# barbararoessle/e2e_multi_view_matching

Measured on NVIDIA H100. Metric: view-tuples/sec @1024 kpts 5-view, higher is better.
Workload: dtype f32 via split operands on the tensor cores (fp16x3 / tf32x3, fp32-faithful) / f64 pose kernels

## Files before the change

e2e_multi_view_matching_b200/csrc/attention_h3.cu:

```cuda
#include "attention_wg.cuh"

int g_attn_h3_variant = 1;
extern "C" void mvm_debug_set_attention_h3_variant(int v) { g_attn_h3_variant = v ? 1 : 0; }

int launch_attention_h3(const float* qkv, const __half* kh, const __half* kl, const __half* vh, const __half* vl,
                        float* out, int batch, int n_pad, AttnSegs segs, int is_cross, cudaStream_t stream) {
  MVM_REQUIRE(qkv && kh && kl && vh && vl && out);
  MVM_REQUIRE(n_pad % 64 == 0 && attn_segs_valid(segs, n_pad, is_cross));
  MvmProfScope prof__(MVM_TAG_ATTN, stream);
  const long long rows = (long long)batch * segs.n_views * n_pad;
  const CUtensorMap* tK = mvm_get_tmap_2d_f16(kh, rows, 256, 256, attn_wg::Cfg<16>::BKV);
  const CUtensorMap* tKlo = mvm_get_tmap_2d_f16(kl, rows, 256, 256, attn_wg::Cfg<16>::BKV);
  const CUtensorMap* tV = mvm_get_tmap_2d_f16(vh, rows, 256, 256, attn_wg::Cfg<16>::BKV);
  const CUtensorMap* tVlo = mvm_get_tmap_2d_f16(vl, rows, 256, 256, attn_wg::Cfg<16>::BKV);
  return attn_wg::launch<16>(tK, tV, tKlo, tVlo, qkv, out, batch, n_pad, segs, is_cross, stream);
}
```

e2e_multi_view_matching_b200/csrc/attention_tc.cu:

```cuda
#include "attention_wg.cuh"

long long* g_attn_dbg = nullptr;

extern "C" void mvm_debug_set_attention_timing(long long* buf) { g_attn_dbg = buf; }

int launch_attention_tc(const float* qkv, const float* vt, float* out, int batch, int n_pad, AttnSegs segs,
                        int is_cross, int n_pass, cudaStream_t stream, const float* klo, const float* vtlo) {
  MVM_REQUIRE(n_pad % 64 == 0 && attn_segs_valid(segs, n_pad, is_cross));
  MvmProfScope prof__(MVM_TAG_ATTN, stream);
  const int V = batch * segs.n_views;
  const long long rows = (long long)V * n_pad;
  const CUtensorMap* tK = mvm_get_tmap_2d(qkv, rows, 768, 768, attn_wg::Cfg<1>::BKV);
  const CUtensorMap* tV = mvm_get_tmap_2d(vt, (long long)V * 256, n_pad, n_pad, attn_wg::HD);
  if (n_pass == 3) {
    MVM_REQUIRE(klo && vtlo);
    const CUtensorMap* tKlo = mvm_get_tmap_2d(klo, rows, 256, 256, attn_wg::Cfg<1>::BKV);
    const CUtensorMap* tVlo = mvm_get_tmap_2d(vtlo, (long long)V * 256, n_pad, n_pad, attn_wg::HD);
    return attn_wg::launch<3>(tK, tV, tKlo, tVlo, qkv, out, batch, n_pad, segs, is_cross, stream);
  }
  return attn_wg::launch<1>(tK, tV, tK, tV, qkv, out, batch, n_pad, segs, is_cross, stream);
}
```

e2e_multi_view_matching_b200/csrc/attention_wg.cuh:

```cuda
#pragma once
#include <cuda_fp16.h>
#include "common.cuh"
#include "kernels.cuh"
#include "tc_common.cuh"

namespace attn_wg {

constexpr int BQ = 128, HD = 64;
constexpr int PRODUCER_WARP = 8;
constexpr int NTHREADS = 384;
constexpr int PRODUCER_REGS = 40, CONSUMER_REGS = 232;
constexpr int PP_BAR = 1;

template <int MODE>
struct Cfg {
  static constexpr bool F16 = MODE == 16;
  static constexpr bool PIPE = F16;
  static constexpr int BKV = F16 ? 128 : 64;
  static constexpr int PL = MODE == 1 ? 1 : 2;
  static constexpr int PLANE = 16384;
  static constexpr int TILE = PL * PLANE;
  static constexpr int ST = MODE == 1 ? 4 : 3;
  static constexpr int OFF_V = ST * TILE;
  static constexpr int OFF_BAR = 2 * ST * TILE;
  static constexpr int SMEM_BYTES = OFF_BAR + 256 + 1024;
};

struct Args {
  const float* qkv;
  float* out;
  int n_pad;
  AttnSegs segs;
  int is_cross;
};

__device__ __forceinline__ float ex2_ftz(float x) {
  float y;
  asm("ex2.approx.ftz.f32 %0, %1;" : "=f"(y) : "f"(x));
  return y;
}
__device__ __forceinline__ float tf32_hi(float x) {
  return __uint_as_float((__float_as_uint(x) + 0x1000u) & 0xffffe000u);
}
__device__ __forceinline__ void split_pack(float x0, float x1, uint32_t& hi, uint32_t& lo) {
  const __half2 h = __floats2half2_rn(x0, x1);
  const float2 hf = __half22float2(h);
  const __half2 l = __floats2half2_rn(x0 - hf.x, x1 - hf.y);
  hi = *reinterpret_cast<const uint32_t*>(&h);
  lo = *reinterpret_cast<const uint32_t*>(&l);
}
__device__ __forceinline__ void named_bar_sync(int id, int n) {
  asm volatile("bar.sync %0, %1;" ::"r"(id), "r"(n) : "memory");
}
__device__ __forceinline__ void named_bar_arrive(int id, int n) {
  asm volatile("bar.arrive %0, %1;" ::"r"(id), "r"(n) : "memory");
}
template <int N>
__device__ __forceinline__ void fence_regs(uint32_t (*a)[4]) {
#pragma unroll
  for (int i = 0; i < N; ++i)
#pragma unroll
    for (int e = 0; e < 4; ++e) asm volatile("" : "+r"(a[i][e])::"memory");
}

template <int MODE>
__global__ void __launch_bounds__(NTHREADS, 1)
attention_wg_kernel(const __grid_constant__ CUtensorMap tmK, const __grid_constant__ CUtensorMap tmV,
                    const __grid_constant__ CUtensorMap tmKlo, const __grid_constant__ CUtensorMap tmVlo,
                    const __grid_constant__ Args g) {
  using C_ = Cfg<MODE>;
  constexpr bool F16 = C_::F16, PIPE = C_::PIPE;
  constexpr int ST = C_::ST, PLANE = C_::PLANE, TILE = C_::TILE, BKV = C_::BKV;
  constexpr int KS = F16 ? 4 : 8;
  constexpr int KP = BKV / (F16 ? 16 : 8);
  constexpr int NSC = BKV / 2;
  extern __shared__ uint8_t smem_raw[];
  uint8_t* smem = reinterpret_cast<uint8_t*>((reinterpret_cast<uintptr_t>(smem_raw) + 1023) & ~uintptr_t(1023));
  uint64_t* bars = reinterpret_cast<uint64_t*>(smem + C_::OFF_BAR);
  uint64_t* k_full = bars;
  uint64_t* k_empty = bars + ST;
  uint64_t* v_full = bars + 2 * ST;
  uint64_t* v_empty = bars + 3 * ST;

  const int warp = threadIdx.x >> 5, lane = threadIdx.x & 31;
  const int q0 = blockIdx.x * BQ;
  const int h = blockIdx.y;
  const int v = blockIdx.z;
  const int T = g.segs.n_views;
  const int t = v % T, b = v / T;
  if (q0 >= g.segs.counts[t]) return;

  if (threadIdx.x == 0) {
    for (int i = 0; i < ST; ++i) {
      tc::mbar_init(k_full + i, 1); tc::mbar_init(k_empty + i, 256);
      tc::mbar_init(v_full + i, 1); tc::mbar_init(v_empty + i, 256);
    }
    tc::fence_barrier_init();
  }
  __syncthreads();

  if (warp >= PRODUCER_WARP) {
    asm volatile("setmaxnreg.dec.sync.aligned.u32 %0;" ::"n"(PRODUCER_REGS));
    if (warp == PRODUCER_WARP && lane == 0) {
      tc::prefetch_tmap(&tmK); tc::prefetch_tmap(&tmV);
      if (MODE != 1) { tc::prefetch_tmap(&tmKlo); tc::prefetch_tmap(&tmVlo); }
      int j = 0;
      for (int sg = 0; sg < T; ++sg) {
        if (g.is_cross ? (sg == t) : (sg != t)) continue;
        const int cnt = g.segs.counts[sg];
        for (int k0 = 0; k0 < cnt; k0 += BKV, ++j) {
          const int s = j % ST;
          const uint32_t ph = ((j / ST) & 1) ^ 1;
          const int krow = (b * T + sg) * g.n_pad + k0;
          uint8_t* sk = smem + s * TILE;
          uint8_t* sv = smem + C_::OFF_V + s * TILE;
          tc::mbar_wait(k_empty + s, ph);
          tc::mbar_arrive_expect_tx(k_full + s, TILE);
          if (F16) {
            tc::tma_load_2d(sk, &tmK, k_full + s, h * HD, krow);
            tc::tma_load_2d(sk + PLANE, &tmKlo, k_full + s, h * HD, krow);
          } else {
            tc::tma_load_2d(sk, &tmK, k_full + s, 256 + h * HD, krow);
            tc::tma_load_2d(sk + 8192, &tmK, k_full + s, 256 + h * HD + 32, krow);
            if (MODE == 3) {
              tc::tma_load_2d(sk + PLANE, &tmKlo, k_full + s, h * HD, krow);
              tc::tma_load_2d(sk + PLANE + 8192, &tmKlo, k_full + s, h * HD + 32, krow);
            }
          }
          tc::mbar_wait(v_empty + s, ph);
          tc::mbar_arrive_expect_tx(v_full + s, TILE);
          if (F16) {
            tc::tma_load_2d(sv, &tmV, v_full + s, h * HD, krow);
            tc::tma_load_2d(sv + PLANE, &tmVlo, v_full + s, h * HD, krow);
          } else {
            const int vrow = (b * T + sg) * 256 + h * HD;
            tc::tma_load_2d(sv, &tmV, v_full + s, k0, vrow);
            tc::tma_load_2d(sv + 8192, &tmV, v_full + s, k0 + 32, vrow);
            if (MODE == 3) {
              tc::tma_load_2d(sv + PLANE, &tmVlo, v_full + s, k0, vrow);
              tc::tma_load_2d(sv + PLANE + 8192, &tmVlo, v_full + s, k0 + 32, vrow);
            }
          }
        }
      }
    }
    return;
  }

  asm volatile("setmaxnreg.inc.sync.aligned.u32 %0;" ::"n"(CONSUMER_REGS));
  const int wg = warp >> 2, wq = warp & 3;
  const int gr = lane >> 2, tq = lane & 3;
  const int lrow = wg * 64 + wq * 16 + gr;
  float2 qraw[KS][4];
  {
    const long long total = (long long)gridDim.z * g.n_pad;
    const long long r0 = (long long)v * g.n_pad + q0 + lrow;
    const float* q_r0 = g.qkv + r0 * 768 + h * HD;
    const float* q_r1 = q_r0 + 8 * 768;
    const bool in0 = r0 < total, in1 = r0 + 8 < total;
    const float2 z = make_float2(0.f, 0.f);
#pragma unroll
    for (int kk = 0; kk < KS; ++kk) {
      if (F16) {
        const int c = 16 * kk + 2 * tq;
        qraw[kk][0] = in0 ? __ldg(reinterpret_cast<const float2*>(q_r0 + c)) : z;
        qraw[kk][1] = in1 ? __ldg(reinterpret_cast<const float2*>(q_r1 + c)) : z;
        qraw[kk][2] = in0 ? __ldg(reinterpret_cast<const float2*>(q_r0 + c + 8)) : z;
        qraw[kk][3] = in1 ? __ldg(reinterpret_cast<const float2*>(q_r1 + c + 8)) : z;
      } else {
        const int c = 8 * kk + tq;
        qraw[kk][0] = make_float2(in0 ? __ldg(q_r0 + c) : 0.f, 0.f);
        qraw[kk][1] = make_float2(in1 ? __ldg(q_r1 + c) : 0.f, 0.f);
        qraw[kk][2] = make_float2(in0 ? __ldg(q_r0 + c + 4) : 0.f, 0.f);
        qraw[kk][3] = make_float2(in1 ? __ldg(q_r1 + c + 4) : 0.f, 0.f);
      }
    }
  }
  uint32_t qhi[KS][4], qlo[KS][4];
  if constexpr (F16) {
#pragma unroll
    for (int kk = 0; kk < KS; ++kk)
#pragma unroll
      for (int e = 0; e < 4; ++e) split_pack(qraw[kk][e].x, qraw[kk][e].y, qhi[kk][e], qlo[kk][e]);
  }

  float o[32];
#pragma unroll
  for (int i = 0; i < 32; ++i) o[i] = 0.f;
  float m_run[2] = {-INFINITY, -INFINITY}, l_run[2] = {0.f, 0.f};
  const float scale_l2e = 0.125f * 1.4426950408889634f;
  const int srcA = (lane & ~3) | (tq >> 1), srcB = srcA + 2;
  float sc[NSC], fo[2];
  uint32_t phi[KP][4], plo[KP][4];

  auto prep_s = [&] {
    if constexpr (!F16) {
#pragma unroll
      for (int kk = 0; kk < KS; ++kk) {
#pragma unroll
        for (int e = 0; e < 4; ++e) {
          float x = qraw[kk][e].x;
          asm volatile("" : "+f"(x));
          const float hi = MODE == 3 ? tf32_hi(x) : x;
          qhi[kk][e] = __float_as_uint(hi);
          qlo[kk][e] = __float_as_uint(MODE == 3 ? tf32_hi(x - hi) : 0.f);
        }
      }
    }
#pragma unroll
    for (int i = 0; i < NSC; ++i) sc[i] = 0.f;
    tc::fence_acc<BKV>(sc);
  };
  auto issue_s = [&](int st, uint32_t ph) {
    tc::mbar_wait(k_full + st, ph);
    const uint32_t kb = tc::smem_u32(smem + st * TILE);
    tc::wgmma_fence();
#pragma unroll
    for (int kk = 0; kk < KS; ++kk) {
      if (F16) {
        const uint64_t dk = tc::make_sw128_desc(kb + kk * 32);
        tc::wgmma_f16_rs<BKV, 0>(sc, qhi[kk], dk);
        tc::wgmma_f16_rs<BKV, 0>(sc, qhi[kk], tc::make_sw128_desc(kb + PLANE + kk * 32));
        tc::wgmma_f16_rs<BKV, 0>(sc, qlo[kk], dk);
      } else {
        const uint32_t off = (kk >> 2) * 8192 + (kk & 3) * 32;
        const uint64_t dk = tc::make_sw128_desc(kb + off);
        tc::wgmma_tf32_rs<64>(sc, qhi[kk], dk);
        if (MODE == 3) {
          tc::wgmma_tf32_rs<64>(sc, qhi[kk], tc::make_sw128_desc(kb + PLANE + off));
          tc::wgmma_tf32_rs<64>(sc, qlo[kk], dk);
        }
      }
    }
    tc::wgmma_commit();
  };
  auto retire_s = [&](int st) {
    tc::fence_acc<BKV>(sc);
    fence_regs<KS>(qhi);
    fence_regs<KS>(qlo);
    tc::mbar_arrive(k_empty + st);
  };
  auto issue_pv = [&](int st, uint32_t ph) {
    tc::mbar_wait(v_full + st, ph);
    const uint32_t vb = tc::smem_u32(smem + C_::OFF_V + st * TILE);
    tc::wgmma_fence();
#pragma unroll
    for (int kk = 0; kk < KP; ++kk) {
      if (F16) {
        const uint64_t dv = tc::make_sw128_desc(vb + kk * 2048);
        tc::wgmma_f16_rs<64, 1>(o, phi[kk], dv);
        tc::wgmma_f16_rs<64, 1>(o, phi[kk], tc::make_sw128_desc(vb + PLANE + kk * 2048));
        tc::wgmma_f16_rs<64, 1>(o, plo[kk], dv);
      } else {
        const uint32_t off = (kk >> 2) * 8192 + (kk & 3) * 32;
        const uint64_t dv = tc::make_sw128_desc(vb + off);
        tc::wgmma_tf32_rs<64>(o, phi[kk], dv);
        if (MODE == 3) {
          tc::wgmma_tf32_rs<64>(o, phi[kk], tc::make_sw128_desc(vb + PLANE + off));
          tc::wgmma_tf32_rs<64>(o, plo[kk], dv);
        }
      }
    }
    tc::wgmma_commit();
  };
  auto retire_pv = [&](int st) {
    tc::fence_acc<64>(o);
    fence_regs<KP>(phi);
    fence_regs<KP>(plo);
    tc::mbar_arrive(v_empty + st);
  };
  auto softmax = [&](int nvalid) {
    if (nvalid < BKV) {
#pragma unroll
      for (int i = 0; i < BKV / 8; ++i) {
        const int key = 8 * i + 2 * tq;
        if (key >= nvalid) { sc[4 * i] = -INFINITY; sc[4 * i + 2] = -INFINITY; }
        if (key + 1 >= nvalid) { sc[4 * i + 1] = -INFINITY; sc[4 * i + 3] = -INFINITY; }
      }
    }
#pragma unroll
    for (int hh = 0; hh < 2; ++hh) {
      float mx = sc[2 * hh];
#pragma unroll
      for (int i = 0; i < BKV / 8; ++i) mx = fmaxf(mx, fmaxf(sc[4 * i + 2 * hh], sc[4 * i + 2 * hh + 1]));
      mx = fmaxf(mx, __shfl_xor_sync(0xffffffffu, mx, 1));
      mx = fmaxf(mx, __shfl_xor_sync(0xffffffffu, mx, 2));
      mx *= scale_l2e;
      fo[hh] = 1.f;
      if (mx > m_run[hh] + 8.f) {
        fo[hh] = ex2_ftz(m_run[hh] - mx);
        m_run[hh] = mx;
        l_run[hh] *= fo[hh];
      }
      const float nm = 7.f - m_run[hh];
      float rs = 0.f;
#pragma unroll
      for (int i = 0; i < BKV / 8; ++i) {
        const float p0 = ex2_ftz(fmaf(sc[4 * i + 2 * hh], scale_l2e, nm));
        const float p1 = ex2_ftz(fmaf(sc[4 * i + 2 * hh + 1], scale_l2e, nm));
        sc[4 * i + 2 * hh] = p0;
        sc[4 * i + 2 * hh + 1] = p1;
        rs += p0 + p1;
      }
      l_run[hh] += rs;
    }
  };
  auto rescale_o = [&] {
#pragma unroll
    for (int hh = 0; hh < 2; ++hh) {
      if (fo[hh] != 1.f) {
#pragma unroll
        for (int i = 0; i < 8; ++i) {
          o[4 * i + 2 * hh] *= fo[hh];
          o[4 * i + 2 * hh + 1] *= fo[hh];
        }
      }
    }
  };
  auto split_p = [&] {
#pragma unroll
    for (int kk = 0; kk < KP; ++kk) {
      if (F16) {
#pragma unroll
        for (int e = 0; e < 4; ++e) split_pack(sc[8 * kk + 2 * e], sc[8 * kk + 2 * e + 1], phi[kk][e], plo[kk][e]);
      } else {
        float a[4];
        const bool odd = tq & 1;
        const float x0 = __shfl_sync(0xffffffffu, sc[4 * kk], srcA), x1 = __shfl_sync(0xffffffffu, sc[4 * kk + 1], srcA);
        const float y0 = __shfl_sync(0xffffffffu, sc[4 * kk + 2], srcA), y1 = __shfl_sync(0xffffffffu, sc[4 * kk + 3], srcA);
        const float z0 = __shfl_sync(0xffffffffu, sc[4 * kk], srcB), z1 = __shfl_sync(0xffffffffu, sc[4 * kk + 1], srcB);
        const float w0 = __shfl_sync(0xffffffffu, sc[4 * kk + 2], srcB), w1 = __shfl_sync(0xffffffffu, sc[4 * kk + 3], srcB);
        a[0] = odd ? x1 : x0; a[1] = odd ? y1 : y0; a[2] = odd ? z1 : z0; a[3] = odd ? w1 : w0;
#pragma unroll
        for (int e = 0; e < 4; ++e) {
          const float hi = MODE == 3 ? tf32_hi(a[e]) : a[e];
          phi[kk][e] = __float_as_uint(hi);
          plo[kk][e] = __float_as_uint(a[e] - hi);
        }
      }
    }
  };

  auto finish_pv = [&](int jn) {
    tc::wgmma_wait<0>();
    tc::fence_acc<64>(o);
    fence_regs<KP>(phi);
    fence_regs<KP>(plo);
    if (jn >= 2) tc::mbar_arrive(v_empty + (jn - 2) % ST);
    if (jn >= 1) {
      rescale_o();
      split_p();
    }
  };
  if (PIPE && wg == 1) named_bar_arrive(PP_BAR + 0, 256);
  int j = 0;
  for (int sg = 0; sg < T; ++sg) {
    if (g.is_cross ? (sg == t) : (sg != t)) continue;
    const int cnt = g.segs.counts[sg];
    for (int k0 = 0; k0 < cnt; k0 += BKV, ++j) {
      const int nvalid = cnt - k0;
      const int s = j % ST;
      const uint32_t ph = (j / ST) & 1;
      if constexpr (PIPE) {
        finish_pv(j);
        prep_s();
        named_bar_sync(PP_BAR + wg, 256);
        if (j == 0) {
          issue_s(s, ph);
          named_bar_arrive(PP_BAR + (wg ^ 1), 256);
          tc::wgmma_wait<0>();
        } else {
          issue_s(s, ph);
          issue_pv((j - 1) % ST, ((j - 1) / ST) & 1);
          named_bar_arrive(PP_BAR + (wg ^ 1), 256);
          tc::wgmma_wait<1>();
        }
        retire_s(s);
        softmax(nvalid);
      } else {
        prep_s();
        issue_s(s, ph);
        tc::wgmma_wait<0>();
        retire_s(s);
        softmax(nvalid);
        rescale_o();
        split_p();
        issue_pv(s, ph);
        tc::wgmma_wait<0>();
        retire_pv(s);
      }
    }
  }
  if constexpr (PIPE) {
    finish_pv(j);
    named_bar_sync(PP_BAR + wg, 256);
    if (j > 0) issue_pv((j - 1) % ST, ((j - 1) / ST) & 1);
    if (wg == 0) named_bar_arrive(PP_BAR + 1, 256);
    tc::wgmma_wait<0>();
    if (j > 0) retire_pv((j - 1) % ST);
  }

#pragma unroll
  for (int hh = 0; hh < 2; ++hh) {
    float l = l_run[hh];
    l += __shfl_xor_sync(0xffffffffu, l, 1);
    l += __shfl_xor_sync(0xffffffffu, l, 2);
    const float inv = 1.f / l;
    const int r = lrow + 8 * hh;
    if (q0 + r < g.n_pad) {
      float* op = g.out + ((long long)v * g.n_pad + q0 + r) * 256 + h * HD + 2 * tq;
#pragma unroll
      for (int i = 0; i < 8; ++i)
        *reinterpret_cast<float2*>(op + 8 * i) = make_float2(o[4 * i + 2 * hh] * inv, o[4 * i + 2 * hh + 1] * inv);
    }
  }
}

template <int MODE>
int launch(const CUtensorMap* tK, const CUtensorMap* tV, const CUtensorMap* tKlo, const CUtensorMap* tVlo, const float* qkv,
           float* out, int batch, int n_pad, const AttnSegs& segs, int is_cross, cudaStream_t stream) {
  using C_ = Cfg<MODE>;
  if (!tK || !tV || !tKlo || !tVlo) return MVM_ERR_LAUNCH;
  mvm_once_per_device(MODE == 16 ? MVM_ONCE_ATTN_H3 : MVM_ONCE_ATTN_TC + 16 * (MODE == 3), [&] {
    cudaFuncSetAttribute(attention_wg_kernel<MODE>, cudaFuncAttributeMaxDynamicSharedMemorySize, C_::SMEM_BYTES);
  });
  Args g;
  g.qkv = qkv; g.out = out; g.n_pad = n_pad; g.segs = segs; g.is_cross = is_cross;
  dim3 grid(mvm_div_up(n_pad, BQ), 4, batch * segs.n_views);
  attention_wg_kernel<MODE><<<grid, NTHREADS, C_::SMEM_BYTES, stream>>>(*tK, *tV, *tKlo, *tVlo, g);
  MVM_CHECK_LAUNCH();
  return MVM_OK;
}

}
```

Baseline: 215.3.

## Make attention kernel persistent with TMA-loaded Q tiles and cross-item KV pipelining

Replaces the one-CTA-per-(query block, head, view) grid with a persistent grid sized to the SM count that strides over work items. Q tiles are now fetched by the producer warp via TMA into a swizzled shared buffer instead of per-thread global loads. The K/V stage counter runs continuously across items, so loads for the next item can overlap the previous item's tail, and the final PV of one item is drained before the next begins. This is meant to remove launch/tail waves and Q-load latency. In exchange it adds shared memory and extra barrier bookkeeping, and static round-robin item assignment may load-balance poorly across uneven segments.

```diff
diff --git a/e2e_multi_view_matching_b200/csrc/attention_h3.cu b/e2e_multi_view_matching_b200/csrc/attention_h3.cu
--- a/e2e_multi_view_matching_b200/csrc/attention_h3.cu
+++ b/e2e_multi_view_matching_b200/csrc/attention_h3.cu
@@ -13,5 +13,6 @@
   const CUtensorMap* tKlo = mvm_get_tmap_2d_f16(kl, rows, 256, 256, attn_wg::Cfg<16>::BKV);
   const CUtensorMap* tV = mvm_get_tmap_2d_f16(vh, rows, 256, 256, attn_wg::Cfg<16>::BKV);
   const CUtensorMap* tVlo = mvm_get_tmap_2d_f16(vl, rows, 256, 256, attn_wg::Cfg<16>::BKV);
-  return attn_wg::launch<16>(tK, tV, tKlo, tVlo, qkv, out, batch, n_pad, segs, is_cross, stream);
+  const CUtensorMap* tQ = mvm_get_tmap_2d(qkv, rows, 768, 768, attn_wg::BQ);
+  return attn_wg::launch<16>(tK, tV, tKlo, tVlo, tQ, qkv, out, batch, n_pad, segs, is_cross, stream);
 }
diff --git a/e2e_multi_view_matching_b200/csrc/attention_tc.cu b/e2e_multi_view_matching_b200/csrc/attention_tc.cu
--- a/e2e_multi_view_matching_b200/csrc/attention_tc.cu
+++ b/e2e_multi_view_matching_b200/csrc/attention_tc.cu
@@ -12,11 +12,12 @@
   const long long rows = (long long)V * n_pad;
   const CUtensorMap* tK = mvm_get_tmap_2d(qkv, rows, 768, 768, attn_wg::Cfg<1>::BKV);
   const CUtensorMap* tV = mvm_get_tmap_2d(vt, (long long)V * 256, n_pad, n_pad, attn_wg::HD);
+  const CUtensorMap* tQ = mvm_get_tmap_2d(qkv, rows, 768, 768, attn_wg::BQ);
   if (n_pass == 3) {
     MVM_REQUIRE(klo && vtlo);
     const CUtensorMap* tKlo = mvm_get_tmap_2d(klo, rows, 256, 256, attn_wg::Cfg<1>::BKV);
     const CUtensorMap* tVlo = mvm_get_tmap_2d(vtlo, (long long)V * 256, n_pad, n_pad, attn_wg::HD);
-    return attn_wg::launch<3>(tK, tV, tKlo, tVlo, qkv, out, batch, n_pad, segs, is_cross, stream);
+    return attn_wg::launch<3>(tK, tV, tKlo, tVlo, tQ, qkv, out, batch, n_pad, segs, is_cross, stream);
   }
-  return attn_wg::launch<1>(tK, tV, tK, tV, qkv, out, batch, n_pad, segs, is_cross, stream);
+  return attn_wg::launch<1>(tK, tV, tK, tV, tQ, qkv, out, batch, n_pad, segs, is_cross, stream);
 }
diff --git a/e2e_multi_view_matching_b200/csrc/attention_wg.cuh b/e2e_multi_view_matching_b200/csrc/attention_wg.cuh
--- a/e2e_multi_view_matching_b200/csrc/attention_wg.cuh
+++ b/e2e_multi_view_matching_b200/csrc/attention_wg.cuh
@@ -22,8 +22,11 @@
   static constexpr int TILE = PL * PLANE;
   static constexpr int ST = MODE == 1 ? 4 : 3;
   static constexpr int OFF_V = ST * TILE;
-  static constexpr int OFF_BAR = 2 * ST * TILE;
+  static constexpr int OFF_Q = 2 * ST * TILE;
+  static constexpr int QBOX = BQ * 32 * 4;
+  static constexpr int OFF_BAR = OFF_Q + 2 * QBOX;
   static constexpr int SMEM_BYTES = OFF_BAR + 256 + 1024;
+  static_assert(SMEM_BYTES <= 232448, "attention: dynamic shared memory above the sm_90 opt-in");
 };
 
 struct Args {
@@ -32,7 +35,20 @@
   int n_pad;
   AttnSegs segs;
   int is_cross;
+  int n_qb;
+  int n_items;
 };
+
+struct Item { int q0, h, v, t, b; };
+__device__ __forceinline__ bool item_at(const Args& g, int it, Item& w) {
+  const int r = it / g.n_qb;
+  w.q0 = (it - r * g.n_qb) * BQ;
+  w.h = r & 3;
+  w.v = r >> 2;
+  w.t = w.v % g.segs.n_views;
+  w.b = w.v / g.segs.n_views;
+  return w.q0 < g.segs.counts[w.t];
+}
 
 __device__ __forceinline__ float ex2_ftz(float x) {
   float y;
@@ -67,34 +83,33 @@
 __global__ void __launch_bounds__(NTHREADS, 1)
 attention_wg_kernel(const __grid_constant__ CUtensorMap tmK, const __grid_constant__ CUtensorMap tmV,
                     const __grid_constant__ CUtensorMap tmKlo, const __grid_constant__ CUtensorMap tmVlo,
-                    const __grid_constant__ Args g) {
+                    const __grid_constant__ CUtensorMap tmQ, const __grid_constant__ Args g) {
   using C_ = Cfg<MODE>;
   constexpr bool F16 = C_::F16, PIPE = C_::PIPE;
-  constexpr int ST = C_::ST, PLANE = C_::PLANE, TILE = C_::TILE, BKV = C_::BKV;
+  constexpr int ST = C_::ST, PLANE = C_::PLANE, TILE = C_::TILE, BKV = C_::BKV, QBOX = C_::QBOX;
   constexpr int KS = F16 ? 4 : 8;
   constexpr int KP = BKV / (F16 ? 16 : 8);
   constexpr int NSC = BKV / 2;
   extern __shared__ uint8_t smem_raw[];
   uint8_t* smem = reinterpret_cast<uint8_t*>((reinterpret_cast<uintptr_t>(smem_raw) + 1023) & ~uintptr_t(1023));
+  uint8_t* sq = smem + C_::OFF_Q;
   uint64_t* bars = reinterpret_cast<uint64_t*>(smem + C_::OFF_BAR);
   uint64_t* k_full = bars;
   uint64_t* k_empty = bars + ST;
   uint64_t* v_full = bars + 2 * ST;
   uint64_t* v_empty = bars + 3 * ST;
+  uint64_t* q_full = bars + 4 * ST;
+  uint64_t* q_empty = bars + 4 * ST + 1;
 
   const int warp = threadIdx.x >> 5, lane = threadIdx.x & 31;
-  const int q0 = blockIdx.x * BQ;
-  const int h = blockIdx.y;
-  const int v = blockIdx.z;
   const int T = g.segs.n_views;
-  const int t = v % T, b = v / T;
-  if (q0 >= g.segs.counts[t]) return;
 
   if (threadIdx.x == 0) {
     for (int i = 0; i < ST; ++i) {
       tc::mbar_init(k_full + i, 1); tc::mbar_init(k_empty + i, 256);
       tc::mbar_init(v_full + i, 1); tc::mbar_init(v_empty + i, 256);
     }
+    tc::mbar_init(q_full, 1); tc::mbar_init(q_empty, 256);
     tc::fence_barrier_init();
   }
   __syncthreads();
@@ -102,43 +117,51 @@
   if (warp >= PRODUCER_WARP) {
     asm volatile("setmaxnreg.dec.sync.aligned.u32 %0;" ::"n"(PRODUCER_REGS));
     if (warp == PRODUCER_WARP && lane == 0) {
-      tc::prefetch_tmap(&tmK); tc::prefetch_tmap(&tmV);
+      tc::prefetch_tmap(&tmK); tc::prefetch_tmap(&tmV); tc::prefetch_tmap(&tmQ);
       if (MODE != 1) { tc::prefetch_tmap(&tmKlo); tc::prefetch_tmap(&tmVlo); }
-      int j = 0;
-      for (int sg = 0; sg < T; ++sg) {
-        if (g.is_cross ? (sg == t) : (sg != t)) continue;
-        const int cnt = g.segs.counts[sg];
-        for (int k0 = 0; k0 < cnt; k0 += BKV, ++j) {
-          const int s = j % ST;
-          const uint32_t ph = ((j / ST) & 1) ^ 1;
-          const int krow = (b * T + sg) * g.n_pad + k0;
-          uint8_t* sk = smem + s * TILE;
-          uint8_t* sv = smem + C_::OFF_V + s * TILE;
-          tc::mbar_wait(k_empty + s, ph);
-          tc::mbar_arrive_expect_tx(k_full + s, TILE);
-          if (F16) {
-            tc::tma_load_2d(sk, &tmK, k_full + s, h * HD, krow);
-            tc::tma_load_2d(sk + PLANE, &tmKlo, k_full + s, h * HD, krow);
-          } else {
-            tc::tma_load_2d(sk, &tmK, k_full + s, 256 + h * HD, krow);
-            tc::tma_load_2d(sk + 8192, &tmK, k_full + s, 256 + h * HD + 32, krow);
-            if (MODE == 3) {
-              tc::tma_load_2d(sk + PLANE, &tmKlo, k_full + s, h * HD, krow);
-              tc::tma_load_2d(sk + PLANE + 8192, &tmKlo, k_full + s, h * HD + 32, krow);
+      int j = 0, qi = 0;
+      for (int it = blockIdx.x; it < g.n_items; it += gridDim.x) {
+        Item w;
+        if (!item_at(g, it, w)) continue;
+        tc::mbar_wait(q_empty, (qi++ & 1) ^ 1);
+        tc::mbar_arrive_expect_tx(q_full, 2 * QBOX);
+        tc::tma_load_2d(sq, &tmQ, q_full, w.h * HD, w.v * g.n_pad + w.q0);
+        tc::tma_load_2d(sq + QBOX, &tmQ, q_full, w.h * HD + 32, w.v * g.n_pad + w.q0);
+        for (int sg = 0; sg < T; ++sg) {
+          if (g.is_cross ? (sg == w.t) : (sg != w.t)) continue;
+          const int cnt = g.segs.counts[sg];
+          for (int k0 = 0; k0 < cnt; k0 += BKV, ++j) {
+            const int s = j % ST;
+            const uint32_t ph = ((j / ST) & 1) ^ 1;
+            const int krow = (w.b * T + sg) * g.n_pad + k0;
+            uint8_t* sk = smem + s * TILE;
+            uint8_t* sv = smem + C_::OFF_V + s * TILE;
+            tc::mbar_wait(k_empty + s, ph);
+            tc::mbar_arrive_expect_tx(k_full + s, TILE);
+            if (F16) {
+              tc::tma_load_2d(sk, &tmK, k_full + s, w.h * HD, krow);
+              tc::tma_load_2d(sk + PLANE, &tmKlo, k_full + s, w.h * HD, krow);
+            } else {
+              tc::tma_load_2d(sk, &tmK, k_full + s, 256 + w.h * HD, krow);
+              tc::tma_load_2d(sk + 8192, &tmK, k_full + s, 256 + w.h * HD + 32, krow);
+              if (MODE == 3) {
+                tc::tma_load_2d(sk + PLANE, &tmKlo, k_full + s, w.h * HD, krow);
+                tc::tma_load_2d(sk + PLANE + 8192, &tmKlo, k_full + s, w.h * HD + 32, krow);
+              }
             }
-          }
-          tc::mbar_wait(v_empty + s, ph);
-          tc::mbar_arrive_expect_tx(v_full + s, TILE);
-          if (F16) {
-            tc::tma_load_2d(sv, &tmV, v_full + s, h * HD, krow);
-            tc::tma_load_2d(sv + PLANE, &tmVlo, v_full + s, h * HD, krow);
-          } else {
-            const int vrow = (b * T + sg) * 256 + h * HD;
-            tc::tma_load_2d(sv, &tmV, v_full + s, k0, vrow);
-            tc::tma_load_2d(sv + 8192, &tmV, v_full + s, k0 + 32, vrow);
-            if (MODE == 3) {
-              tc::tma_load_2d(sv + PLANE, &tmVlo, v_full + s, k0, vrow);
-              tc::tma_load_2d(sv + PLANE + 8192, &tmVlo, v_full + s, k0 + 32, vrow);
+            tc::mbar_wait(v_empty + s, ph);
+            tc::mbar_arrive_expect_tx(v_full + s, TILE);
+            if (F16) {
+              tc::tma_load_2d(sv, &tmV, v_full + s, w.h * HD, krow);
+              tc::tma_load_2d(sv + PLANE, &tmVlo, v_full + s, w.h * HD, krow);
+            } else {
+              const int vrow = (w.b * T + sg) * 256 + w.h * HD;
+              tc::tma_load_2d(sv, &tmV, v_full + s, k0, vrow);
+              tc::tma_load_2d(sv + 8192, &tmV, v_full + s, k0 + 32, vrow);
+              if (MODE == 3) {
+                tc::tma_load_2d(sv + PLANE, &tmVlo, v_full + s, k0, vrow);
+                tc::tma_load_2d(sv + PLANE + 8192, &tmVlo, v_full + s, k0 + 32, vrow);
+              }
             }
           }
         }
@@ -151,43 +174,34 @@
   const int wg = warp >> 2, wq = warp & 3;
   const int gr = lane >> 2, tq = lane & 3;
   const int lrow = wg * 64 + wq * 16 + gr;
-  float2 qraw[KS][4];
-  {
-    const long long total = (long long)gridDim.z * g.n_pad;
-    const long long r0 = (long long)v * g.n_pad + q0 + lrow;
-    const float* q_r0 = g.qkv + r0 * 768 + h * HD;
-    const float* q_r1 = q_r0 + 8 * 768;
-    const bool in0 = r0 < total, in1 = r0 + 8 < total;
-    const float2 z = make_float2(0.f, 0.f);
-#pragma unroll
-    for (int kk = 0; kk < KS; ++kk) {
-      if (F16) {
-        const int c = 16 * kk + 2 * tq;
-        qraw[kk][0] = in0 ? __ldg(reinterpret_cast<const float2*>(q_r0 + c)) : z;
-        qraw[kk][1] = in1 ? __ldg(reinterpret_cast<const float2*>(q_r1 + c)) : z;
-        qraw[kk][2] = in0 ? __ldg(reinterpret_cast<const float2*>(q_r0 + c + 8)) : z;
-        qraw[kk][3] = in1 ? __ldg(reinterpret_cast<const float2*>(q_r1 + c + 8)) : z;
-      } else {
-        const int c = 8 * kk + tq;
-        qraw[kk][0] = make_float2(in0 ? __ldg(q_r0 + c) : 0.f, 0.f);
-        qraw[kk][1] = make_float2(in1 ? __ldg(q_r1 + c) : 0.f, 0.f);
-        qraw[kk][2] = make_float2(in0 ? __ldg(q_r0 + c + 4) : 0.f, 0.f);
-        qraw[kk][3] = make_float2(in1 ? __ldg(q_r1 + c + 4) : 0.f, 0.f);
-      }
-    }
-  }
   uint32_t qhi[KS][4], qlo[KS][4];
-  if constexpr (F16) {
+  auto q_frag = [&](int kk, int e) -> const float* {
+    int sw = gr;
+    asm volatile("" : "+r"(sw));
+    const int r = lrow + 8 * (e & 1);
+    const int c = F16 ? 16 * kk + 2 * tq + 8 * (e >> 1) : 8 * kk + tq + 4 * (e >> 1);
+    return reinterpret_cast<const float*>(sq + (c >> 5) * QBOX + r * 128 + ((((c & 31) >> 2) ^ sw) << 4) + (c & 3) * 4);
+  };
+  auto load_q16 = [&](uint32_t ph) {
+    tc::mbar_wait(q_full, ph);
 #pragma unroll
     for (int kk = 0; kk < KS; ++kk)
 #pragma unroll
-      for (int e = 0; e < 4; ++e) split_pack(qraw[kk][e].x, qraw[kk][e].y, qhi[kk][e], qlo[kk][e]);
-  }
-
-  float o[32];
-#pragma unroll
-  for (int i = 0; i < 32; ++i) o[i] = 0.f;
-  float m_run[2] = {-INFINITY, -INFINITY}, l_run[2] = {0.f, 0.f};
+      for (int e = 0; e < 4; ++e) {
+        const float2 x = *reinterpret_cast<const float2*>(q_frag(kk, e));
+        split_pack(x.x, x.y, qhi[kk][e], qlo[kk][e]);
+      }
+    tc::mbar_arrive(q_empty);
+  };
+
+  float o[32], m_run[2], l_run[2];
+  auto reset_o = [&] {
+#pragma unroll
+    for (int i = 0; i < 32; ++i) o[i] = 0.f;
+#pragma unroll
+    for (int hh = 0; hh < 2; ++hh) { m_run[hh] = -INFINITY; l_run[hh] = 0.f; }
+  };
+  reset_o();
   const float scale_l2e = 0.125f * 1.4426950408889634f;
   const int srcA = (lane & ~3) | (tq >> 1), srcB = srcA + 2;
   float sc[NSC], fo[2];
@@ -199,7 +213,7 @@
       for (int kk = 0; kk < KS; ++kk) {
 #pragma unroll
         for (int e = 0; e < 4; ++e) {
-          float x = qraw[kk][e].x;
+          float x = *q_frag(kk, e);
           asm volatile("" : "+f"(x));
           const float hi = MODE == 3 ? tf32_hi(x) : x;
           qhi[kk][e] = __float_as_uint(hi);
@@ -341,93 +355,131 @@
     }
   };
 
-  auto finish_pv = [&](int jn) {
+  auto store_o = [&](int it) {
+    Item w;
+    item_at(g, it, w);
+#pragma unroll
+    for (int hh = 0; hh < 2; ++hh) {
+      float l = l_run[hh];
+      l += __shfl_xor_sync(0xffffffffu, l, 1);
+      l += __shfl_xor_sync(0xffffffffu, l, 2);
+      const float inv = 1.f / l;
+      const int r = lrow + 8 * hh;
+      if (w.q0 + r < g.n_pad) {
+        float* op = g.out + ((long long)w.v * g.n_pad + w.q0 + r) * 256 + w.h * HD + 2 * tq;
+#pragma unroll
+        for (int i = 0; i < 8; ++i)
+          *reinterpret_cast<float2*>(op + 8 * i) = make_float2(o[4 * i + 2 * hh] * inv, o[4 * i + 2 * hh + 1] * inv);
+      }
+    }
+  };
+
+  auto finish_pv = [&](int jn, int Jn) {
     tc::wgmma_wait<0>();
     tc::fence_acc<64>(o);
     fence_regs<KP>(phi);
     fence_regs<KP>(plo);
-    if (jn >= 2) tc::mbar_arrive(v_empty + (jn - 2) % ST);
+    if (jn >= 2) tc::mbar_arrive(v_empty + (Jn - 2) % ST);
     if (jn >= 1) {
       rescale_o();
       split_p();
     }
   };
   if (PIPE && wg == 1) named_bar_arrive(PP_BAR + 0, 256);
-  int j = 0;
-  for (int sg = 0; sg < T; ++sg) {
-    if (g.is_cross ? (sg == t) : (sg != t)) continue;
-    const int cnt = g.segs.counts[sg];
-    for (int k0 = 0; k0 < cnt; k0 += BKV, ++j) {
-      const int nvalid = cnt - k0;
-      const int s = j % ST;
-      const uint32_t ph = (j / ST) & 1;
-      if constexpr (PIPE) {
-        finish_pv(j);
-        prep_s();
-        named_bar_sync(PP_BAR + wg, 256);
-        if (j == 0) {
+  int J = 0, j = 0, qi = 0;
+  int cur = -1;
+  for (int it = blockIdx.x; it < g.n_items; it += gridDim.x) {
+    Item w;
+    if (!item_at(g, it, w)) continue;
+    if (PIPE && cur >= 0) {
+      finish_pv(j, J);
+      named_bar_sync(PP_BAR + wg, 256);
+      issue_pv((J - 1) % ST, ((J - 1) / ST) & 1);
+      named_bar_arrive(PP_BAR + (wg ^ 1), 256);
+      tc::wgmma_wait<0>();
+      retire_pv((J - 1) % ST);
+      store_o(cur);
+    }
+    cur = it;
+    if constexpr (PIPE) {
+      tc::wgmma_wait<0>();
+      load_q16(qi++ & 1);
+    } else {
+      tc::mbar_wait(q_full, qi++ & 1);
+    }
+    reset_o();
+    j = 0;
+    for (int sg = 0; sg < T; ++sg) {
+      if (g.is_cross ? (sg == w.t) : (sg != w.t)) continue;
+      const int cnt = g.segs.counts[sg];
+      for (int k0 = 0; k0 < cnt; k0 += BKV, ++j, ++J) {
+        const int nvalid = cnt - k0;
+        const int s = J % ST;
+        const uint32_t ph = (J / ST) & 1;
+        if constexpr (PIPE) {
+          finish_pv(j, J);
+          prep_s();
+          named_bar_sync(PP_BAR + wg, 256);
+          if (j == 0) {
+            issue_s(s, ph);
+            named_bar_arrive(PP_BAR + (wg ^ 1), 256);
+            tc::wgmma_wait<0>();
+          } else {
+            issue_s(s, ph);
+            issue_pv((J - 1) % ST, ((J - 1) / ST) & 1);
+            named_bar_arrive(PP_BAR + (wg ^ 1), 256);
+            tc::wgmma_wait<1>();
+          }
+          retire_s(s);
+          softmax(nvalid);
+        } else {
+          prep_s();
           issue_s(s, ph);
-          named_bar_arrive(PP_BAR + (wg ^ 1), 256);
           tc::wgmma_wait<0>();
-        } else {
-          issue_s(s, ph);
-          issue_pv((j - 1) % ST, ((j - 1) / ST) & 1);
-          named_bar_arrive(PP_BAR + (wg ^ 1), 256);
-          tc::wgmma_wait<1>();
-        }
-        retire_s(s);
-        softmax(nvalid);
-      } else {
-        prep_s();
-        issue_s(s, ph);
-        tc::wgmma_wait<0>();
-        retire_s(s);
-        softmax(nvalid);
-        rescale_o();
-        split_p();
-        issue_pv(s, ph);
-        tc::wgmma_wait<0>();
-        retire_pv(s);
-      }
+          retire_s(s);
+          softmax(nvalid);
+          rescale_o();
+          split_p();
+          issue_pv(s, ph);
+          tc::wgmma_wait<0>();
+          retire_pv(s);
+        }
+      }
+    }
+    if constexpr (!PIPE) {
+      tc::mbar_arrive(q_empty);
+      store_o(cur);
     }
   }
   if constexpr (PIPE) {
-    finish_pv(j);
+    finish_pv(j, J);
     named_bar_sync(PP_BAR + wg, 256);
-    if (j > 0) issue_pv((j - 1) % ST, ((j - 1) / ST) & 1);
+    if (cur >= 0) issue_pv((J - 1) % ST, ((J - 1) / ST) & 1);
     if (wg == 0) named_bar_arrive(PP_BAR + 1, 256);
     tc::wgmma_wait<0>();
-    if (j > 0) retire_pv((j - 1) % ST);
+    if (cur >= 0) {
+      retire_pv((J - 1) % ST);
+      store_o(cur);
+    }
   }
-
-#pragma unroll
-  for (int hh = 0; hh < 2; ++hh) {
-    float l = l_run[hh];
-    l += __shfl_xor_sync(0xffffffffu, l, 1);
-    l += __shfl_xor_sync(0xffffffffu, l, 2);
-    const float inv = 1.f / l;
-    const int r = lrow + 8 * hh;
-    if (q0 + r < g.n_pad) {
-      float* op = g.out + ((long long)v * g.n_pad + q0 + r) * 256 + h * HD + 2 * tq;
-#pragma unroll
-      for (int i = 0; i < 8; ++i)
-        *reinterpret_cast<float2*>(op + 8 * i) = make_float2(o[4 * i + 2 * hh] * inv, o[4 * i + 2 * hh + 1] * inv);
-    }
-  }
 }
 
 template <int MODE>
-int launch(const CUtensorMap* tK, const CUtensorMap* tV, const CUtensorMap* tKlo, const CUtensorMap* tVlo, const float* qkv,
-           float* out, int batch, int n_pad, const AttnSegs& segs, int is_cross, cudaStream_t stream) {
+int launch(const CUtensorMap* tK, const CUtensorMap* tV, const CUtensorMap* tKlo, const CUtensorMap* tVlo,
+           const CUtensorMap* tQ, const float* qkv, float* out, int batch, int n_pad, const AttnSegs& segs, int is_cross,
+           cudaStream_t stream) {
   using C_ = Cfg<MODE>;
-  if (!tK || !tV || !tKlo || !tVlo) return MVM_ERR_LAUNCH;
+  if (!tK || !tV || !tKlo || !tVlo || !tQ) return MVM_ERR_LAUNCH;
   mvm_once_per_device(MODE == 16 ? MVM_ONCE_ATTN_H3 : MVM_ONCE_ATTN_TC + 16 * (MODE == 3), [&] {
     cudaFuncSetAttribute(attention_wg_kernel<MODE>, cudaFuncAttributeMaxDynamicSharedMemorySize, C_::SMEM_BYTES);
   });
   Args g;
   g.qkv = qkv; g.out = out; g.n_pad = n_pad; g.segs = segs; g.is_cross = is_cross;
-  dim3 grid(mvm_div_up(n_pad, BQ), 4, batch * segs.n_views);
-  attention_wg_kernel<MODE><<<grid, NTHREADS, C_::SMEM_BYTES, stream>>>(*tK, *tV, *tKlo, *tVlo, g);
+  g.n_qb = mvm_div_up(n_pad, BQ);
+  g.n_items = g.n_qb * 4 * batch * segs.n_views;
+  if (g.n_items <= 0) return MVM_OK;
+  const int grid = std::min(g.n_items, mvm_dev_info().n_sm);
+  attention_wg_kernel<MODE><<<grid, NTHREADS, C_::SMEM_BYTES, stream>>>(*tK, *tV, *tKlo, *tVlo, *tQ, g);
   MVM_CHECK_LAUNCH();
   return MVM_OK;
 }
```

After: 219.1 (median of 6 runs). +1.8%, better.
